# mpkuse/rgbd_odometry

Hardware: NVIDIA B200
Metric: frame-pairs aligned/s (640x480, 4-lvl) (higher is better)
Workload: dtype f32+f64

## Files before the change

### rgbd_odometry_b200/_lib.py

```python
import ctypes as C
import os

from . import build as _build

MAX_LEVELS = 6
STAGES = ["h2d", "pyramid", "canny", "edt_rows", "normgrad", "solve", "d2h"]


class Config(C.Structure):
    _fields_ = [("width", C.c_int), ("height", C.c_int), ("levels", C.c_int), ("max_batch", C.c_int), ("device", C.c_int),
                ("keep_now_depth", C.c_int), ("trace_iters", C.c_int)]


class SolverParams(C.Structure):
    _fields_ = [("solver", C.c_int), ("jacobian", C.c_int), ("weight", C.c_int), ("arithmetic", C.c_int),
                ("huber_k", C.c_float), ("lm_lambda0", C.c_double), ("iters", C.c_int * MAX_LEVELS), ("residual", C.c_int)]


class PairInfo(C.Structure):
    _fields_ = [("status", C.c_int), ("npts", C.c_int * MAX_LEVELS), ("best_index", C.c_int * MAX_LEVELS),
                ("iterations_run", C.c_int * MAX_LEVELS), ("best_energy", C.c_float * MAX_LEVELS),
                ("visible_ratio", C.c_float * MAX_LEVELS), ("laplacian_b", C.c_float)]


class CovInfo(C.Structure):
    _fields_ = [("status", C.c_int), ("level", C.c_int), ("nvis", C.c_int), ("sigma2", C.c_double), ("logdet", C.c_double)]


class PhotoConfig(C.Structure):
    _fields_ = [("width", C.c_int), ("height", C.c_int), ("levels", C.c_int), ("max_batch", C.c_int), ("device", C.c_int)]


class PhotoInfo(C.Structure):
    _fields_ = [("status", C.c_int), ("iters_run", C.c_int), ("nreproj", C.c_int), ("sumsq_first", C.c_double),
                ("sumsq_last", C.c_double), ("visible", C.c_double), ("A", C.c_double * 36), ("b", C.c_double * 6)]


class KeyframePolicy(C.Structure):
    _fields_ = [("keyframe_every", C.c_int), ("use_quality_gates", C.c_int), ("laplacian_thresh", C.c_float),
                ("visible_ratio_thresh", C.c_float), ("min_reprojections", C.c_int)]


RGBD_MAX_LEVELS = 5


class RgbdConfig(C.Structure):
    _fields_ = [("width", C.c_int), ("height", C.c_int), ("levels", C.c_int), ("max_batch", C.c_int), ("device", C.c_int)]


class RgbdParams(C.Structure):
    _fields_ = [("iterations", C.c_int), ("gradient_threshold", C.c_int), ("min_points", C.c_int), ("max_points", C.c_int),
                ("eps_norm_exit", C.c_double)]


class RgbdInfo(C.Structure):
    _fields_ = [("status", C.c_int), ("npts", C.c_int * RGBD_MAX_LEVELS), ("iters_run", C.c_int * RGBD_MAX_LEVELS),
                ("updates", C.c_int * RGBD_MAX_LEVELS), ("nvis_last", C.c_int * RGBD_MAX_LEVELS),
                ("eps_norm_first", C.c_double * RGBD_MAX_LEVELS), ("eps_norm_last", C.c_double * RGBD_MAX_LEVELS)]


SYMBOLS = [
    "dvo_last_error", "dvo_device_count", "dvo_create", "dvo_destroy", "dvo_set_stream", "dvo_synchronize",
    "dvo_set_intrinsics", "dvo_set_frames", "dvo_set_frames_raw", "dvo_promote_now_to_ref", "dvo_build_pyramids", "dvo_prepare",
    "dvo_set_initial_pose", "dvo_run", "dvo_process", "dvo_join", "dvo_join_stream", "dvo_get_poses", "dvo_align_batch", "dvo_level_dims", "dvo_get_level_buffer",
    "dvo_get_points", "dvo_eval_normal_equations", "dvo_eval_normal_equations_ex", "dvo_get_trace", "dvo_get_energies", "dvo_enable_timing", "dvo_get_stage_ms",
    "dvo_launch_count", "dvo_gop_compose", "dvo_run_sequences", "dvo_run_sequences_gated", "dvo_run_sequences_mem",
    "dvo_pose_covariance", "dvo_run_sequences_cov",
    "dvo_photo_create", "dvo_photo_destroy", "dvo_photo_set_stream", "dvo_photo_synchronize", "dvo_photo_launch_count",
    "dvo_photo_set_intrinsics", "dvo_photo_set_frames", "dvo_photo_prepare_ref", "dvo_photo_set_pose", "dvo_photo_estimate",
    "dvo_photo_get_poses", "dvo_photo_get_level", "dvo_photo_get_A", "dvo_photo_eval", "dvo_photo_put_level",
    "dvo_blob_create", "dvo_blob_upload", "dvo_blob_download", "dvo_blob_device_ptr", "dvo_blob_bytes", "dvo_blob_destroy",
    "dvo_undistort",
    "dvo_rgbd_create", "dvo_rgbd_destroy", "dvo_rgbd_set_stream", "dvo_rgbd_synchronize", "dvo_rgbd_launch_count",
    "dvo_rgbd_set_intrinsics", "dvo_rgbd_set_frames", "dvo_rgbd_compute_jacobians", "dvo_rgbd_set_pose", "dvo_rgbd_gauss_newton",
    "dvo_rgbd_get_poses", "dvo_rgbd_level_dims", "dvo_rgbd_get_level", "dvo_rgbd_get_A", "dvo_rgbd_eval",
]

_lib = None


def load(build_if_missing=True):
    global _lib
    if _lib is not None:
        return _lib
    path = _build.LIB
    if build_if_missing:
        path = _build.build_cuda()
    if not os.path.exists(path):
        raise RuntimeError(f"{path} is missing: build it with `python -m rgbd_odometry_b200.build` (no CPU fallback exists)")
    lib = C.CDLL(path)
    lib.dvo_last_error.restype = C.c_char_p
    lib.dvo_launch_count.restype = C.c_longlong
    lib.dvo_launch_count.argtypes = [C.c_void_p]
    lib.dvo_create.argtypes = [C.POINTER(Config), C.POINTER(C.c_void_p)]
    lib.dvo_destroy.argtypes = [C.c_void_p]
    lib.dvo_set_stream.argtypes = [C.c_void_p, C.c_void_p]
    lib.dvo_synchronize.argtypes = [C.c_void_p]
    lib.dvo_set_intrinsics.argtypes = [C.c_void_p, C.c_float, C.c_float, C.c_float, C.c_float]
    lib.dvo_set_frames.argtypes = [C.c_void_p, C.c_int, C.c_int, C.c_int, C.c_void_p, C.c_void_p, C.c_int]
    lib.dvo_set_frames_raw.argtypes = [C.c_void_p, C.c_int, C.c_int, C.c_int, C.c_void_p, C.c_void_p, C.c_int]
    lib.dvo_promote_now_to_ref.argtypes = [C.c_void_p, C.c_int, C.c_int]
    lib.dvo_build_pyramids.argtypes = [C.c_void_p, C.c_int, C.c_int, C.c_int]
    lib.dvo_prepare.argtypes = [C.c_void_p, C.c_int, C.c_int, C.c_int]
    lib.dvo_set_initial_pose.argtypes = [C.c_void_p, C.c_int, C.c_int, C.c_void_p, C.c_int]
    lib.dvo_run.argtypes = [C.c_void_p, C.c_int, C.c_int, C.POINTER(SolverParams)]
    lib.dvo_process.argtypes = [C.c_void_p, C.c_int, C.c_int, C.POINTER(SolverParams), C.c_void_p]
    lib.dvo_join.argtypes = [C.c_void_p]
    lib.dvo_join_stream.argtypes = [C.c_void_p, C.c_void_p]
    lib.dvo_get_poses.argtypes = [C.c_void_p, C.c_int, C.c_int, C.c_void_p, C.c_void_p, C.c_int]
    lib.dvo_align_batch.argtypes = [C.c_void_p, C.c_int, C.c_void_p, C.c_void_p, C.c_void_p, C.c_void_p,
                                    C.POINTER(SolverParams), C.c_void_p, C.c_void_p]
    lib.dvo_level_dims.argtypes = [C.c_void_p, C.c_int, C.POINTER(C.c_int), C.POINTER(C.c_int)]
    lib.dvo_get_level_buffer.argtypes = [C.c_void_p, C.c_int, C.c_int, C.c_int, C.c_int, C.c_void_p, C.c_size_t]
    lib.dvo_get_points.argtypes = [C.c_void_p, C.c_int, C.c_int, C.c_void_p, C.c_void_p, C.c_void_p, C.c_int, C.POINTER(C.c_int)]
    lib.dvo_eval_normal_equations.argtypes = [C.c_void_p, C.c_int, C.c_int, C.c_void_p, C.c_int, C.c_int, C.c_int, C.c_float,
                                              C.c_void_p, C.c_void_p, C.POINTER(C.c_double), C.POINTER(C.c_int),
                                              C.c_void_p, C.c_void_p, C.c_void_p, C.c_void_p, C.c_void_p]
    lib.dvo_eval_normal_equations_ex.argtypes = [C.c_void_p, C.c_int, C.c_int, C.c_void_p, C.POINTER(SolverParams),
                                                 C.c_void_p, C.c_void_p, C.POINTER(C.c_double), C.POINTER(C.c_int),
                                                 C.c_void_p, C.c_void_p, C.c_void_p, C.c_void_p, C.c_void_p]
    lib.dvo_get_trace.argtypes = [C.c_void_p, C.c_int, C.c_int, C.c_void_p]
    lib.dvo_get_energies.argtypes = [C.c_void_p, C.c_int, C.c_int, C.c_void_p, C.c_int]
    lib.dvo_enable_timing.argtypes = [C.c_void_p, C.c_int]
    lib.dvo_get_stage_ms.argtypes = [C.c_void_p, C.c_void_p]
    lib.dvo_gop_compose.argtypes = [C.c_void_p, C.c_int, C.c_int, C.c_void_p, C.c_void_p, C.c_void_p, C.c_int]
    lib.dvo_run_sequences.argtypes = [C.c_void_p, C.c_int, C.c_int, C.c_void_p, C.c_void_p, C.POINTER(SolverParams), C.c_int,
                                      C.c_void_p, C.c_void_p, C.c_void_p]
    lib.dvo_run_sequences_gated.argtypes = [C.c_void_p, C.c_int, C.c_int, C.c_void_p, C.c_void_p, C.POINTER(SolverParams),
                                            C.POINTER(KeyframePolicy), C.c_void_p, C.c_void_p, C.c_void_p, C.c_void_p]
    lib.dvo_run_sequences_mem.argtypes = [C.c_void_p, C.c_int, C.c_int, C.c_void_p, C.c_void_p, C.c_int, C.POINTER(SolverParams),
                                          C.POINTER(KeyframePolicy), C.c_void_p, C.c_void_p, C.c_void_p, C.c_void_p]
    lib.dvo_pose_covariance.argtypes = [C.c_void_p, C.c_int, C.c_int, C.POINTER(SolverParams), C.c_int, C.c_void_p, C.c_void_p, C.c_int]
    lib.dvo_run_sequences_cov.argtypes = [C.c_void_p, C.c_int, C.c_int, C.c_void_p, C.c_void_p, C.c_int, C.POINTER(SolverParams),
                                          C.POINTER(KeyframePolicy), C.c_void_p, C.c_void_p, C.c_void_p, C.c_void_p, C.c_void_p, C.c_void_p]
    lib.dvo_photo_create.argtypes = [C.POINTER(PhotoConfig), C.POINTER(C.c_void_p)]
    lib.dvo_photo_destroy.argtypes = [C.c_void_p]
    lib.dvo_photo_set_stream.argtypes = [C.c_void_p, C.c_void_p]
    lib.dvo_photo_synchronize.argtypes = [C.c_void_p]
    lib.dvo_photo_launch_count.restype = C.c_longlong
    lib.dvo_photo_launch_count.argtypes = [C.c_void_p]
    lib.dvo_photo_set_intrinsics.argtypes = [C.c_void_p, C.c_double, C.c_double, C.c_double, C.c_double]
    lib.dvo_photo_set_frames.argtypes = [C.c_void_p, C.c_int, C.c_int, C.c_int, C.c_void_p, C.c_void_p, C.c_int]
    lib.dvo_photo_prepare_ref.argtypes = [C.c_void_p, C.c_int, C.c_int, C.c_int]
    lib.dvo_photo_set_pose.argtypes = [C.c_void_p, C.c_int, C.c_int, C.c_void_p]
    lib.dvo_photo_estimate.argtypes = [C.c_void_p, C.c_int, C.c_int, C.c_int, C.c_int, C.c_int, C.c_double, C.c_double]
    lib.dvo_photo_get_poses.argtypes = [C.c_void_p, C.c_int, C.c_int, C.c_void_p, C.c_void_p]
    lib.dvo_photo_get_level.argtypes = [C.c_void_p, C.c_int, C.c_int, C.c_int, C.c_int, C.c_void_p, C.c_size_t, C.c_int]
    lib.dvo_photo_get_A.argtypes = [C.c_void_p, C.c_int, C.c_int, C.c_void_p]
    lib.dvo_photo_put_level.argtypes = [C.c_void_p, C.c_int, C.c_int, C.c_int, C.c_int, C.c_void_p, C.c_size_t]
    lib.dvo_blob_create.argtypes = [C.c_size_t, C.c_int, C.POINTER(C.c_void_p)]
    lib.dvo_blob_upload.argtypes = [C.c_void_p, C.c_void_p, C.c_size_t]
    lib.dvo_blob_download.argtypes = [C.c_void_p, C.c_void_p, C.c_size_t]
    lib.dvo_blob_device_ptr.argtypes = [C.c_void_p]
    lib.dvo_blob_device_ptr.restype = C.c_void_p
    lib.dvo_blob_bytes.argtypes = [C.c_void_p]
    lib.dvo_blob_bytes.restype = C.c_size_t
    lib.dvo_blob_destroy.argtypes = [C.c_void_p]
    lib.dvo_photo_eval.argtypes = [C.c_void_p, C.c_int, C.c_int, C.c_void_p, C.c_int, C.c_double, C.c_void_p, C.c_void_p,
                                   C.POINTER(C.c_double), C.POINTER(C.c_int), C.POINTER(C.c_int), C.c_void_p]
    lib.dvo_undistort.argtypes = [C.c_void_p, C.c_void_p, C.c_int, C.c_int, C.c_int, C.c_int, C.c_void_p, C.c_void_p, C.c_int, C.c_void_p]
    lib.dvo_rgbd_create.argtypes = [C.POINTER(RgbdConfig), C.POINTER(C.c_void_p)]
    lib.dvo_rgbd_destroy.argtypes = [C.c_void_p]
    lib.dvo_rgbd_set_stream.argtypes = [C.c_void_p, C.c_void_p]
    lib.dvo_rgbd_synchronize.argtypes = [C.c_void_p]
    lib.dvo_rgbd_launch_count.restype = C.c_longlong
    lib.dvo_rgbd_launch_count.argtypes = [C.c_void_p]
    lib.dvo_rgbd_set_intrinsics.argtypes = [C.c_void_p, C.c_double, C.c_double, C.c_double, C.c_double]
    lib.dvo_rgbd_set_frames.argtypes = [C.c_void_p, C.c_int, C.c_int, C.c_int, C.c_void_p, C.c_void_p, C.c_int]
    lib.dvo_rgbd_compute_jacobians.argtypes = [C.c_void_p, C.c_int, C.c_int, C.c_int]
    lib.dvo_rgbd_set_pose.argtypes = [C.c_void_p, C.c_int, C.c_int, C.c_void_p]
# ... 20 lines not shown
```

### rgbd_odometry_b200/build.py

```python
import os
import shutil
import subprocess

PKG = os.path.dirname(os.path.abspath(__file__))
ROOT = os.path.dirname(PKG)
CSRC = os.path.join(PKG, "csrc")
LIB = os.path.join(PKG, "libdvo_b200.so")
SYNTH_SRC = os.path.join(PKG, "synth", "synth.cpp")
SYNTH_LIB = os.path.join(PKG, "synth", "libdvo_synth.so")
HOST_DIR = os.path.join(PKG, "host")
HOST_LIB = os.path.join(PKG, "libdvo_host.so")


def _nvcc():
    for cand in (shutil.which("nvcc"), "/usr/local/cuda/bin/nvcc"):
        if cand and os.path.exists(cand):
            return cand
    raise RuntimeError("nvcc not found: libdvo_b200.so cannot be built and there is no CPU fallback")


def _stale(target, sources):
    if not os.path.exists(target):
        return True
    t = os.path.getmtime(target)
    return any(os.path.getmtime(s) > t for s in sources)


def cuda_sources():
    srcs = [os.path.join(CSRC, f) for f in sorted(os.listdir(CSRC)) if f.endswith(".cu")]
    deps = [os.path.join(CSRC, f) for f in sorted(os.listdir(CSRC)) if f.endswith(".cuh")]
    deps.append(os.path.join(ROOT, "include", "dvo_b200.h"))
    return srcs, deps


PER_FILE_FLAGS = {"photometric.cu": ["-fmad=false"], "rgbd.cu": ["-fmad=false"], "frontend.cu": ["-fmad=false"]}
COMPILE_FLAGS = ["-gencode", "arch=compute_100a,code=sm_100a", "-lineinfo", "-O3", "-std=c++17", "-Xcompiler", "-fPIC,-ffp-contract=off"]
OBJ_DIR = os.path.join(PKG, "build")


def build_cuda(force=False, verbose=False):
    srcs, deps = cuda_sources()
    os.makedirs(OBJ_DIR, exist_ok=True)
    objs, relink = [], force or not os.path.exists(LIB)
    for src in srcs:
        name = os.path.basename(src)
        obj = os.path.join(OBJ_DIR, name[:-3] + ".o")
        objs.append(obj)
        if force or _stale(obj, [src] + deps):
            extra = os.environ.get("DVO_NVCC_EXTRA", "").split()
            cmd = [_nvcc()] + COMPILE_FLAGS + PER_FILE_FLAGS.get(name, []) + extra + (["-Xptxas", "-v"] if verbose else []) + ["-c", "-o", obj, src]
            subprocess.check_call(cmd, cwd=CSRC)
            relink = True
    if relink or _stale(LIB, objs):
        subprocess.check_call([_nvcc(), "-gencode", "arch=compute_100a,code=sm_100a", "-shared", "-cudart", "static", "-o", LIB] + objs)
    return LIB


def build_synth(force=False):
    if force or _stale(SYNTH_LIB, [SYNTH_SRC]):
        subprocess.check_call(["g++", "-O2", "-std=c++17", "-fPIC", "-shared", "-pthread", "-o", SYNTH_LIB, SYNTH_SRC])
    return SYNTH_LIB


def build_host(force=False):
    if not os.path.isdir(HOST_DIR):
        return None
    srcs = [os.path.join(HOST_DIR, f) for f in sorted(os.listdir(HOST_DIR)) if f.endswith(".cpp")]
    if not srcs:
        return None
    deps = [os.path.join(HOST_DIR, f) for f in sorted(os.listdir(HOST_DIR)) if f.endswith(".h")]
    deps.append(os.path.join(ROOT, "include", "dvo_b200.h"))
    build_cuda()
    if force or _stale(HOST_LIB, srcs + deps + [LIB]):
        cmd = ["g++", "-O2", "-std=c++17", "-fPIC", "-shared", "-I", os.path.join(ROOT, "include"), "-I", HOST_DIR, "-o", HOST_LIB] + srcs + \
              ["-L", PKG, "-ldvo_b200", "-Wl,-rpath,$ORIGIN"]
        subprocess.check_call(cmd)
    return HOST_LIB


def build_all(force=False):
    build_cuda(force)
    build_synth(force)
    build_host(force)


if __name__ == "__main__":
    import sys
    build_all(force="--force" in sys.argv)
    print("built:", LIB)
```

### rgbd_odometry_b200/csrc/preprocess.cu

```cuda
#include <stdlib.h>

#include "common.cuh"

struct PyrArgs {
    PyrGeom g;
    uint8_t* gray;
    uint16_t* depth;
    int first;
    int sub_total;
    int l0;
    const unsigned char* active;
};

__global__ void __launch_bounds__(256) pyramid_nearest_kernel(PyrArgs a) {
    const int b = a.first + blockIdx.y;
    if (a.active && !a.active[b]) return;
    int q = blockIdx.x * blockDim.x + threadIdx.x;
    if (q >= a.sub_total) return;
    int l = a.l0;
    while (l < a.g.L - 1 && q >= a.g.P[l]) { q -= a.g.P[l]; ++l; }
    const int w = a.g.w[l], W0 = a.g.w[0], H0 = a.g.h[0];
    const int y = q / w, x = q - y * w;
    const int sy = min(y << l, H0 - 1), sx = min(x << l, W0 - 1);
    const long long src = lvl_at(a.g, 0, b) + (long long)sy * W0 + sx;
// ... 63 lines not shown
    uint32_t gv[4];
#pragma unroll
    for (int j = 0; j < 4; ++j) gv[j] = a.gray[row + sx[j]];
    if (a.depth) {
        uint32_t dv[4];
#pragma unroll
        for (int j = 0; j < 4; ++j) { dv[j] = a.depth[row + sx[j]]; }
#pragma unroll
        for (int j = 0; j < 4; ++j) dv[j] = dv[j] ? dv[j] : 1u;
        *reinterpret_cast<uint2*>(a.depth + dst) = make_uint2(dv[0] | (dv[1] << 16), dv[2] | (dv[3] << 16));
    }
    *reinterpret_cast<uint32_t*>(a.gray + dst) = gv[0] | (gv[1] << 8) | (gv[2] << 16) | (gv[3] << 24);
}

int launch_pyramid(dvo_ctx* c, int first, int count, int frames_mask) {
    const PyrGeom& g = c->geom;
    if (g.L < 2) return DVO_OK;
    const bool vec1 = (g.w[0] == 2 * g.w[1]) && (g.w[1] % 4 == 0);
    const int l0 = vec1 ? 2 : 1;
    int sub = 0;
    bool vec_rest = true;
    for (int l = l0; l < g.L; ++l) { sub += g.P[l]; vec_rest = vec_rest && (g.w[l] % 4 == 0) && (g.off[l] % 4 == 0) && (g.P[l] % 4 == 0); }
    for (int f = 0; f < 2; ++f) {
        if (!(frames_mask & (1 << f))) continue;
        PyrArgs a; a.g = g; a.gray = c->gray[f]; a.depth = c->depth[f]; a.first = first; a.sub_total = sub; a.l0 = l0; a.active = c->active;
        if (vec1 && g.w[1] % 8 == 0 && g.off[1] % 8 == 0 && g.P[1] % 8 == 0 && g.P[0] % 16 == 0) {
            dim3 grid1((g.P[1] / 8 + 255) / 256, count);
            pyramid_level1_vec8_kernel<<<grid1, 256, 0, c->stream>>>(a);
            c->launches++;
        } else if (vec1) {
            dim3 grid1((g.P[1] / 4 + 255) / 256, count);
            pyramid_level1_vec4_kernel<<<grid1, 256, 0, c->stream>>>(a);
            c->launches++;
        }
        if (sub > 0 && vec_rest) {
            dim3 grid((sub / 4 + 255) / 256, count);
            pyramid_nearest_vec4_kernel<<<grid, 256, 0, c->stream>>>(a);
            c->launches++;
        } else if (sub > 0) {
            dim3 grid((sub + 255) / 256, count);
            pyramid_nearest_kernel<<<grid, 256, 0, c->stream>>>(a);
            c->launches++;
        }
    }
    DVO_CUDA(cudaGetLastError());
    return DVO_OK;
}

struct CannyArgs {
    const uint8_t* gray[2];
    uint8_t* edge[2];
    const uint16_t* depth;
    uint16_t* gcol;
    float *X, *Y, *Z;
    int* pix;
    int* npts;
    unsigned* nedge[2];
    int w, h, P, L;
    int frame0;
    int count;
    long long gscratch_frame_stride;
    float tmpfx, tmpfy, tmpcx, tmpcy;
    uint32_t* gscratch;
    long long gscratch_stride;
    int first;
    int bm_words;
    const unsigned char* active;
};

__device__ __forceinline__ void sobel3(const uint8_t* __restrict__ g, int w, int h, int y, int x, int& dx, int& dy) {
    const int ym = max(y - 1, 0), yp = min(y + 1, h - 1), xm = max(x - 1, 0), xp = min(x + 1, w - 1);
    const uint8_t* r0 = g + ym * w; const uint8_t* r1 = g + y * w; const uint8_t* r2 = g + yp * w;
    const int a = r0[xm], b = r0[x], c = r0[xp], d = r1[xm], f = r1[xp], p = r2[xm], q = r2[x], r = r2[xp];
    dx = (c + 2 * f + r) - (a + 2 * d + p);
    dy = (p + 2 * q + r) - (a + 2 * b + c);
}
__device__ __forceinline__ int mag_at(const uint8_t* __restrict__ g, int w, int h, int y, int x) {
    if ((unsigned)y >= (unsigned)h || (unsigned)x >= (unsigned)w) return 0;
    int dx, dy; sobel3(g, w, h, y, x, dx, dy);
    return dx * dx + dy * dy;
}

__device__ __forceinline__ uint32_t expand4(uint32_t nib) { return (((nib & 0xFu) * 0x00204081u) & 0x01010101u) * 0xFFu; }

__device__ __forceinline__ void row_sums(const uint8_t* __restrict__ grow, int w, int x, int lane, int& hs, int& hb) {
    const int v = (x < w) ? (int)grow[x] : 0;
    int l = __shfl_up_sync(0xffffffffu, v, 1), r = __shfl_down_sync(0xffffffffu, v, 1);
    if (lane == 0) l = (x > 0 && x < w) ? (int)grow[x - 1] : v;
    if (lane == 31) r = (x + 1 < w) ? (int)grow[x + 1] : v;
    if (x + 1 >= w) r = v;
    hs = r - l; hb = l + 2 * v + r;
}

#ifndef DVO_NMS_L2_AHEAD
#define DVO_NMS_L2_AHEAD 4
#endif
#ifndef DVO_NMS_MIN_BLOCKS
#define DVO_NMS_MIN_BLOCKS 2
#endif
#ifndef DVO_NMS_ROWS
#define DVO_NMS_ROWS 48
#endif
#ifndef DVO_NMS_WARPS
#define DVO_NMS_WARPS 8
#endif
constexpr int NMS_ROWS = DVO_NMS_ROWS, NMS_WARPS = DVO_NMS_WARPS;
struct NmsArgs {
    const uint8_t* gray[2];
    uint32_t* scratch;
    long long slot_stride, frame_stride;
    long long off[DVO_MAX_LEVELS];
    long long bm_off[DVO_MAX_LEVELS];
    int w[DVO_MAX_LEVELS], h[DVO_MAX_LEVELS], P[DVO_MAX_LEVELS], bm_words[DVO_MAX_LEVELS];
    int chunks[DVO_MAX_LEVELS], strips[DVO_MAX_LEVELS], task_end[DVO_MAX_LEVELS];
    int L, first, count, frame0;
    float low, high;
    const unsigned char* active;
};
struct NmsSums { float s[4], b[4], sH, bH; };
struct NmsMags { float m[4], L, R; };
struct NmsGrad { float dx[4], dy[4]; };

template <bool VEC>
__global__ void __launch_bounds__(NMS_WARPS * 32, DVO_NMS_MIN_BLOCKS) sobel_nms_kernel(NmsArgs a) {
    const int lane = threadIdx.x & 31;
    int task = blockIdx.x * NMS_WARPS + (threadIdx.x >> 5);
    int l = 0;
    while (l < a.L && task >= a.task_end[l]) ++l;
    if (l >= a.L) return;
    if (l) task -= a.task_end[l - 1];
    const int chunks = a.chunks[l], strips = a.strips[l];
    const int chunk = task % chunks, t2 = task / chunks, strip = t2 % strips, img = t2 / strips;
    const int second = (img >= a.count) ? 1 : 0;
    const int frame = second ? DVO_FRAME_NOW : a.frame0;
    const int b = a.first + img - second * a.count;
    if (a.active && !a.active[b]) return;
    const int w = a.w[l], h = a.h[l];
    const int wd = (w + 31) >> 5, pitch = wd + 2;
    const uint8_t* __restrict__ g = a.gray[frame] + a.off[l] + (long long)b * a.P[l];
    uint32_t* Cb = a.scratch + (long long)b * a.slot_stride + (long long)frame * a.frame_stride + a.bm_off[l];
    const int bmw = a.bm_words[l];
    const int c0 = chunk << 7, xb = c0 + (lane << 2);
    const int y0 = strip * NMS_ROWS, y1 = min(h, y0 + NMS_ROWS);
    const bool first_lane = (lane == 0), last_lane = (lane == 31);
    const bool halo_valid = first_lane ? (c0 > 0) : (last_lane && c0 + 128 < w);
    const bool self_left = (xb == 0), self_right = (xb + 4 >= w);
    const int hx0 = first_lane ? c0 - 2 : c0 + 128;
    const uint32_t sel_near = 0x7440u + (first_lane ? 1u : 0u), sel_far = 0x7440u + (first_lane ? 0u : 1u);
    const float lowt = (xb < w) ? a.low : 3.0e38f, high = a.high;
    const float K = 13573.0f / 32768.0f;

    const bool in_image = (xb < w);
    const uint8_t* __restrict__ gx = g + (in_image ? xb : 0);
    const uint8_t* __restrict__ gh = g + (halo_valid ? hx0 : 0);
    const unsigned roff_max = (unsigned)((h - 1) * w);
    auto load_row = [&](unsigned roff, uint32_t& wv, uint32_t& hv) {
        if (VEC) {
            wv = in_image ? *reinterpret_cast<const uint32_t*>(gx + roff) : 0u;
            hv = halo_valid ? (uint32_t)*reinterpret_cast<const uint16_t*>(gh + roff) : 0u;
        } else {
            const uint8_t* __restrict__ row = g + roff;
            wv = 0u;
#pragma unroll
            for (int j = 0; j < 4; ++j) wv |= (uint32_t)row[min(xb + j, w - 1)] << (8 * j);
            hv = halo_valid ? ((uint32_t)row[hx0] | ((uint32_t)row[min(hx0 + 1, w - 1)] << 8)) : 0u;
        }
    };
    auto byte_f = [](uint32_t wv, uint32_t sel) { return __uint_as_float(__byte_perm(wv, 0x4B000000u, sel)) - 8388608.0f; };
    auto sums = [&](uint32_t wv, uint32_t hv, NmsSums& S) {
        float v[4];
#pragma unroll
        for (int j = 0; j < 4; ++j) v[j] = byte_f(wv, 0x7440u + j);
        const float hn = byte_f(hv, sel_near), hf = byte_f(hv, sel_far);
        float lft = __shfl_up_sync(0xffffffffu, v[3], 1), rgt = __shfl_down_sync(0xffffffffu, v[0], 1);
        if (first_lane) lft = hn;
        if (last_lane) rgt = hn;
        if (self_left) lft = v[0];
        if (self_right) rgt = v[3];
        S.s[0] = v[1] - lft;  S.s[1] = v[2] - v[0]; S.s[2] = v[3] - v[1]; S.s[3] = rgt - v[2];
        S.b[0] = fmaf(2.0f, v[0], lft) + v[1];  S.b[1] = fmaf(2.0f, v[1], v[0]) + v[2];
        S.b[2] = fmaf(2.0f, v[2], v[1]) + v[3]; S.b[3] = fmaf(2.0f, v[3], v[2]) + rgt;
        const float gm1 = first_lane ? hf : v[3], gp1 = first_lane ? v[0] : hf;
        S.sH = gp1 - gm1; S.bH = fmaf(2.0f, hn, gm1) + gp1;
    };
    auto grad_mag = [&](bool inside, const NmsSums& A, const NmsSums& B, const NmsSums& Cs, NmsGrad& G, NmsMags& M) {
        float mH;
        if (inside) {
#pragma unroll
            for (int j = 0; j < 4; ++j) {
                G.dx[j] = fmaf(2.0f, B.s[j], A.s[j]) + Cs.s[j]; G.dy[j] = Cs.b[j] - A.b[j];
                M.m[j] = fmaf(G.dx[j], G.dx[j], G.dy[j] * G.dy[j]);
            }
            const float dxH = fmaf(2.0f, B.sH, A.sH) + Cs.sH, dyH = Cs.bH - A.bH;
            mH = halo_valid ? fmaf(dxH, dxH, dyH * dyH) : 0.0f;
            if (!VEC) {
#pragma unroll
                for (int j = 0; j < 4; ++j) if (xb + j >= w) M.m[j] = 0.0f;
            }
        } else {
#pragma unroll
            for (int j = 0; j < 4; ++j) { G.dx[j] = 0.0f; G.dy[j] = 0.0f; M.m[j] = 0.0f; }
            mH = 0.0f;
        }
        M.L = __shfl_up_sync(0xffffffffu, M.m[3], 1); M.R = __shfl_down_sync(0xffffffffu, M.m[0], 1);
        if (first_lane) M.L = mH;
// ... 4 lines not shown
    uint32_t wv, hv;
    NmsSums S0, S1, S2;
    NmsMags M0, M1, M2;
    NmsGrad G0, G1;
    auto row_off = [&](int r) { return min((unsigned)max(r, 0) * (unsigned)w, roff_max); };
    load_row(row_off(y0 - 2), wv, hv); sums(wv, hv, S0);
    load_row(row_off(y0 - 1), wv, hv); sums(wv, hv, S1);
    load_row(row_off(y0), wv, hv);     sums(wv, hv, S2);
    grad_mag(y0 > 0, S0, S1, S2, G0, M0);
    load_row(row_off(y0 + 1), wv, hv); sums(wv, hv, S0);
    grad_mag(true, S1, S2, S0, G0, M1);
    uint32_t wvn, hvn;
    load_row(row_off(y0 + 2), wvn, hvn);
    unsigned roff_next = row_off(y0 + 3);
    unsigned roff_l2 = row_off(y0 + 3 + DVO_NMS_L2_AHEAD);

    const int widx = (c0 >> 5) + (lane >> 3);
    const bool writer = ((lane & 7) == 0) && widx < wd;
    uint32_t* Cp = Cb + (long long)(y0 + 1) * pitch + 1 + widx;
    const int sh = (lane & 3) << 2;

    auto nms_row = [&](const NmsMags& P, const NmsMags& C, const NmsMags& N, const NmsGrad& Gc) {
        float crm[4], ncm[4];
#pragma unroll
        for (int j = 0; j < 4; ++j) { crm[j] = ((j < 3) ? C.m[j < 3 ? j + 1 : 3] : C.R) - 0.5f; ncm[j] = N.m[j] - 0.5f; }
        uint32_t bits = 0u;
#pragma unroll
        for (int j = 0; j < 4; ++j) {
            const float m = C.m[j];
            const float cl = j ? C.m[j > 0 ? j - 1 : 0] : C.L;
            const float pl = j ? P.m[j > 0 ? j - 1 : 0] : P.L, pr = (j < 3) ? P.m[j < 3 ? j + 1 : 3] : P.R;
            const float nl = j ? N.m[j > 0 ? j - 1 : 0] : N.L, nr = (j < 3) ? N.m[j < 3 ? j + 1 : 3] : N.R;
            const float adx = fabsf(Gc.dx[j]), ady = fabsf(Gc.dy[j]);
            const float t = adx * K, u = fmaf(adx, -2.0f, ady);
            const bool horiz = ady < t, vert = u > t;
            const bool neg = Gc.dx[j] * Gc.dy[j] < 0.0f;
            const float da = neg ? pr : pl, db = neg ? nl : nr;
            const float na = horiz ? cl : (vert ? P.m[j] : da);
            const float nb = horiz ? crm[j] : (vert ? ncm[j] : db);
            const bool cand = (m > na) && (m > nb) && (m > lowt);
            const bool strong = cand && (m > high);
            bits |= (cand ? (1u << j) : 0u) | (strong ? (0x10000u << j) : 0u);
        }
        bits <<= sh;
        bits |= __shfl_xor_sync(0xffffffffu, bits, 1);
        bits |= __shfl_xor_sync(0xffffffffu, bits, 2);
        const uint32_t hi = __shfl_down_sync(0xffffffffu, bits, 4);
        if (writer) {
            Cp[0] = __byte_perm(bits, hi, 0x5410);
            Cp[bmw] = __byte_perm(bits, hi, 0x7632);
        }
        Cp += pitch;
    };
    auto row_step = [&](const NmsSums& A, const NmsSums& B, NmsSums& Cs, const NmsMags& P, const NmsMags& C, NmsMags& N,
                        const NmsGrad& Gc, NmsGrad& Gn) {
        wv = wvn; hv = hvn;
        load_row(roff_next, wvn, hvn); roff_next = min(roff_next + (unsigned)w, roff_max);
        if (DVO_NMS_L2_AHEAD > 0) {
            if (in_image) asm volatile("prefetch.global.L2 [%0];" :: "l"(gx + roff_l2));
            roff_l2 = min(roff_l2 + (unsigned)w, roff_max);
        }
        sums(wv, hv, Cs);
        grad_mag(true, A, B, Cs, Gn, N);
        nms_row(P, C, N, Gc);
    };
    const int yend = (y1 == h) ? y1 - 1 : y1;
    int y = y0;
    for (; y + 6 <= yend; y += 6) {
        row_step(S2, S0, S1, M0, M1, M2, G0, G1);
        row_step(S0, S1, S2, M1, M2, M0, G1, G0);
        row_step(S1, S2, S0, M2, M0, M1, G0, G1);
        row_step(S2, S0, S1, M0, M1, M2, G1, G0);
        row_step(S0, S1, S2, M1, M2, M0, G0, G1);
        row_step(S1, S2, S0, M2, M0, M1, G1, G0);
    }
    for (; y < yend; ++y) {
        row_step(S2, S0, S1, M0, M1, M2, G0, G1);
        S2 = S0; S0 = S1; M0 = M1; M1 = M2; G0 = G1;
    }
    if (y1 == h) {
        grad_mag(false, S2, S0, S1, G1, M2);
        nms_row(M0, M1, M2, G0);
    }
}

constexpr int CANNY_MAX_WARPS = 24;
#ifndef DVO_CANNY_INTERLEAVE
#define DVO_CANNY_INTERLEAVE 1
#endif
#ifndef DVO_CANNY_STOP_AFTER
#define DVO_CANNY_STOP_AFTER 0
#endif

template <bool GLOBAL_BITMAPS> struct HystPtr { typedef volatile uint32_t* type; };
template <> struct HystPtr<true> { typedef uint32_t* type; };

template <bool GLOBAL_BITMAPS>
__global__ void __launch_bounds__(768, 2) canny_kernel(CannyArgs a) {
    extern __shared__ uint32_t smem_u32[];
    __shared__ int s_scan[CANNY_MAX_WARPS + 1];
    __shared__ int s_base;
    __shared__ unsigned s_cnt;
    __shared__ unsigned char s_chg[2][768];
    const int T = blockDim.x;
    const int tid = threadIdx.x, lane = tid & 31, warp = tid >> 5;
#if DVO_CANNY_INTERLEAVE
    const bool both = a.count != 0x7fffffff;
    const int second = both ? (int)(blockIdx.x & 1u) : 0;
    const int frame = second ? DVO_FRAME_NOW : a.frame0;
    const int b = a.first + (both ? (int)(blockIdx.x >> 1) : (int)blockIdx.x);
#else
    const int second = (blockIdx.x >= (unsigned)a.count) ? 1 : 0;
    const int frame = second ? DVO_FRAME_NOW : a.frame0;
    const int b = a.first + (int)blockIdx.x - second * a.count;
#endif
    const bool do_points = (frame == DVO_FRAME_REF), do_cols = (frame == DVO_FRAME_NOW);
    if (a.active && !a.active[b]) return;
    const int w = a.w, h = a.h;
    const int wd = (w + 31) >> 5, pitch = wd + 2;
    const int nwords = a.bm_words;
    uint32_t* C = GLOBAL_BITMAPS ? a.gscratch + (long long)b * a.gscratch_stride + (long long)frame * a.gscratch_frame_stride : smem_u32;
    uint32_t* E = C + nwords;

    if (GLOBAL_BITMAPS) {
        for (int i = tid; i < pitch; i += T) { C[i] = 0u; E[i] = 0u; C[(h + 1) * pitch + i] = 0u; E[(h + 1) * pitch + i] = 0u; }
        for (int y = tid; y < h; y += T) {
            C[(y + 1) * pitch] = 0u; E[(y + 1) * pitch] = 0u; C[(y + 1) * pitch + wd + 1] = 0u; E[(y + 1) * pitch + wd + 1] = 0u;
        }
    } else {
        const uint32_t* __restrict__ src = a.gscratch + (long long)b * a.gscratch_stride + (long long)frame * a.gscratch_frame_stride;
        if ((reinterpret_cast<uintptr_t>(src) & 15) == 0 && (nwords & 1) == 0) {
            const uint4* s4 = reinterpret_cast<const uint4*>(src); uint4* d4 = reinterpret_cast<uint4*>(C);
            for (int i = tid; i < (nwords >> 1); i += T) d4[i] = s4[i];
        } else {
            for (int i = tid; i < 2 * nwords; i += T) C[i] = src[i];
        }
    }
    if (tid == 0) { s_cnt = 0u; s_base = 0; }
    __syncthreads();

#if DVO_CANNY_STOP_AFTER == 1
    return;
#endif
    {
        const int Hs = max(1, min(h, min(T, 768) / wd));
        const int Rh = (h + Hs - 1) / Hs;
        const int items = wd * Hs;
        const int sh = tid / wd, wx = tid - sh * wd;
        const bool owner = tid < items;
        const int ya = sh * Rh, yb = min(h, ya + Rh);
        for (int i = tid; i < 2 * 768; i += T) (&s_chg[0][0])[i] = (i < 768) ? 1 : 0;
        __syncthreads();
        int cur = 0;
        for (;;) {
            int changed = 0;
            bool active = false;
            if (owner && ya < yb) {
                for (int dsy = -1; dsy <= 1 && !active; ++dsy)
                    for (int dwx = -1; dwx <= 1; ++dwx) {
                        const int s2 = sh + dsy, w2 = wx + dwx;
                        if (s2 >= 0 && s2 < Hs && w2 >= 0 && w2 < wd && s_chg[cur][s2 * wd + w2]) { active = true; break; }
                    }
            }
            if (active) {
                auto spread = [](uint32_t l, uint32_t c, uint32_t r) { return c | (c << 1) | (c >> 1) | (l >> 31) | (r << 31); };
                auto flood = [](uint32_t f, uint32_t c) {
                    const uint32_t up = ((c + f) ^ c) & c;
                    const uint32_t cr = __brev(c), fr = __brev(f);
                    return f | up | __brev(((cr + fr) ^ cr) & cr);
                };
                typename HystPtr<GLOBAL_BITMAPS>::type Ev = E;
                const uint32_t* Cv = C;
                {
                    int idx = (ya + 1) * pitch + wx + 1;
                    uint32_t sp = spread(Ev[idx - pitch - 1], Ev[idx - pitch], Ev[idx - pitch + 1]);
                    uint32_t el = Ev[idx - 1], ec = Ev[idx], er = Ev[idx + 1];
                    for (int y = ya; y < yb; ++y, idx += pitch) {
                        const uint32_t nl = Ev[idx + pitch - 1], nc = Ev[idx + pitch], nr = Ev[idx + pitch + 1];
                        const uint32_t c = Cv[idx];
                        uint32_t f = ec;
                        if (c != 0u && ec != c) {
                            f = flood(ec | (c & (sp | spread(el, ec, er) | spread(nl, nc, nr))), c);
                            if (f != ec) { Ev[idx] = f; changed = 1; }
                        }
                        sp = spread(el, f, er); el = nl; ec = nc; er = nr;
                    }
                }
                {
                    int idx = yb * pitch + wx + 1;
                    uint32_t sp = spread(Ev[idx + pitch - 1], Ev[idx + pitch], Ev[idx + pitch + 1]);
                    uint32_t el = Ev[idx - 1], ec = Ev[idx], er = Ev[idx + 1];
                    for (int y = yb - 1; y >= ya; --y, idx -= pitch) {
                        const uint32_t nl = Ev[idx - pitch - 1], nc = Ev[idx - pitch], nr = Ev[idx - pitch + 1];
                        const uint32_t c = Cv[idx];
                        uint32_t f = ec;
                        if (c != 0u && ec != c) {
                            f = flood(ec | (c & (sp | spread(el, ec, er) | spread(nl, nc, nr))), c);
                            if (f != ec) { Ev[idx] = f; changed = 1; }
                        }
                        sp = spread(el, f, er); el = nl; ec = nc; er = nr;
                    }
                }
            }
            if (owner) s_chg[cur ^ 1][tid] = (unsigned char)changed;
            cur ^= 1;
            if (!__syncthreads_or(changed)) break;
        }
    }

#if DVO_CANNY_STOP_AFTER == 2
    return;
#endif
    const int nw = h * wd;
    {
        uint8_t* eo = a.edge[frame] + (long long)b * a.P;
        unsigned cnt = 0;
        const bool vec_ok = (w % 16 == 0) && ((reinterpret_cast<uintptr_t>(eo) & 15) == 0);
        for (int q = tid; q < nw; q += T) {
            const int y = q / wd, wx = q - y * wd;
            const uint32_t e = E[(y + 1) * pitch + wx + 1];
            cnt += __popc(e);
            const int x0 = wx << 5;
            if (vec_ok && x0 + 32 <= w) {
                uint4 v0, v1;
                v0.x = expand4(e); v0.y = expand4(e >> 4); v0.z = expand4(e >> 8); v0.w = expand4(e >> 12);
                v1.x = expand4(e >> 16); v1.y = expand4(e >> 20); v1.z = expand4(e >> 24); v1.w = expand4(e >> 28);
                uint4* dst = reinterpret_cast<uint4*>(eo + (long long)y * w + x0);
                dst[0] = v0; dst[1] = v1;
            } else {
                for (int i = 0; i < 32 && x0 + i < w; ++i) eo[(long long)y * w + x0 + i] = ((e >> i) & 1u) ? 255 : 0;
            }
        }
        for (int o = 16; o > 0; o >>= 1) cnt += __shfl_down_sync(0xffffffffu, cnt, o);
        if (lane == 0 && cnt) atomicAdd(&s_cnt, cnt);
    }

#if DVO_CANNY_STOP_AFTER == 3
    return;
#endif
    if (do_points) {
        const uint16_t* __restrict__ dep = a.depth + (long long)b * a.P;
        for (int q = tid; q < nw; q += T) {
            const int y = q / wd, wx = q - y * wd;
            const int idx = (y + 1) * pitch + wx + 1;
            uint32_t e = E[idx], sel = 0u;
            const uint16_t* __restrict__ dr = dep + (long long)y * w + (wx << 5);
            while (e) {
                const int i0 = __ffs(e) - 1; e &= e - 1;
                const int i1 = e ? __ffs(e) - 1 : i0; e &= e - 1;
                const int i2 = e ? __ffs(e) - 1 : i0; e &= e - 1;
                const int i3 = e ? __ffs(e) - 1 : i0; e &= e - 1;
                const unsigned d0 = dr[i0], d1 = dr[i1], d2 = dr[i2], d3 = dr[i3];
                sel |= (d0 > 100u ? 1u << i0 : 0u) | (d1 > 100u ? 1u << i1 : 0u) | (d2 > 100u ? 1u << i2 : 0u) | (d3 > 100u ? 1u << i3 : 0u);
            }
            E[idx] = sel;
        }
    }
    __syncthreads();
    if (tid == 0) a.nedge[frame][(long long)b * a.L] = s_cnt;

    const int hw = (h + 31) >> 5, hwp = hw | 1;
    uint32_t* Et = C;
    if (do_cols) {
        const int nwarps = T >> 5;
        for (int blk = warp; blk < hw * wd; blk += nwarps) {
            const int wy = blk / wd, wx = blk - wy * wd;
            const int y = (wy << 5) + lane;
            const uint32_t word = (y < h) ? E[(y + 1) * pitch + wx + 1] : 0u;
            uint32_t mine = 0u;
#pragma unroll
            for (int j = 0; j < 32; ++j) { const uint32_t bt = __ballot_sync(0xffffffffu, (word >> j) & 1u); if (lane == j) mine = bt; }
            Et[((wx << 5) + lane) * hwp + wy] = mine;
        }
    }
    __syncthreads();

    if (do_cols) {
        uint16_t* gc = a.gcol + (long long)b * a.P;
        const int BIG = 1 << 20;
        for (int x = tid; x < w; x += T) {
            const uint32_t* col = Et + x * hwp;
            int lastrow = -BIG;
            int nextrow = -1;
            for (int wy = 0; wy < hw; ++wy) {
                const uint32_t Wd = col[wy];
                const int base = wy << 5;
                if (nextrow < base + 32) {
                    nextrow = BIG;
                    for (int kk = wy + 1; kk < hw; ++kk) { const uint32_t vv = col[kk]; if (vv) { nextrow = (kk << 5) + __ffs(vv) - 1; break; } }
                }
                uint16_t* o = gc + (long long)base * w + x;
#pragma unroll
                for (int bt = 0; bt < 32; ++bt) {
                    if (base + bt < h) {
                        const uint32_t mle = Wd & (0xffffffffu >> (31 - bt));
                        const uint32_t mge = Wd & (0xffffffffu << bt);
                        const int dn = mle ? bt - (31 - __clz(mle)) : base + bt - lastrow;
                        const int up = mge ? (__ffs(mge) - 1) - bt : nextrow - (base + bt);
                        o[(long long)bt * w] = (uint16_t)min(min(dn, up), DVO_EDT_INF_1D);
                    }
                }
                if (Wd) lastrow = base + 31 - __clz(Wd);
            }
        }
    }

    if (do_points) {
        const uint16_t* __restrict__ dep = a.depth + (long long)b * a.P;
        float* X = a.X + (long long)b * a.P; float* Y = a.Y + (long long)b * a.P; float* Z = a.Z + (long long)b * a.P;
        int* pix = a.pix + (long long)b * a.P;
        const int per = (nw + T - 1) / T;
        const int q0 = min(nw, tid * per), q1 = min(nw, q0 + per);
        int mycnt = 0;
        for (int q = q0; q < q1; ++q) { const int y = q / wd, wx = q - y * wd; mycnt += __popc(E[(y + 1) * pitch + wx + 1]); }
        int incl = mycnt;
        for (int o = 1; o < 32; o <<= 1) { const int t = __shfl_up_sync(0xffffffffu, incl, o); if (lane >= o) incl += t; }
        if (lane == 31) s_scan[warp] = incl;
        __syncthreads();
        if (tid < 32) {
            const int nwp = T >> 5;
            const int v = (tid < nwp) ? s_scan[tid] : 0;
            int iv = v;
            for (int o = 1; o < 32; o <<= 1) { const int t = __shfl_up_sync(0xffffffffu, iv, o); if (lane >= o) iv += t; }
            if (tid < nwp) s_scan[tid] = iv - v;
            if (tid == 31) s_scan[CANNY_MAX_WARPS] = iv;
        }
        __syncthreads();
        int off = s_scan[warp] + (incl - mycnt);
        for (int q = q0; q < q1; ++q) {
            const int y = q / wd, wx = q - y * wd;
            uint32_t v = E[(y + 1) * pitch + wx + 1];
            const uint16_t* __restrict__ dr = dep + (long long)y * w;
            while (v) {
                int xs[4], n = 0;
#pragma unroll
                for (int k = 0; k < 4; ++k) {
                    if (v) { xs[k] = (wx << 5) + __ffs(v) - 1; v &= v - 1; n = k + 1; } else xs[k] = xs[0];
                }
                unsigned dv[4];
#pragma unroll
                for (int k = 0; k < 4; ++k) dv[k] = dr[xs[k]];
#pragma unroll
                for (int k = 0; k < 4; ++k) {
                    if (k < n) {
                        const int x = xs[k];
                        const float z = __fdiv_rn((float)dv[k], 1000.0f);
                        X[off + k] = __fmul_rn(__fmul_rn(z, __fsub_rn((float)x, a.tmpcx)), a.tmpfx);
                        Y[off + k] = __fmul_rn(__fmul_rn(z, __fsub_rn((float)y, a.tmpcy)), a.tmpfy);
                        Z[off + k] = z;
                        pix[off + k] = y * w + x;
                    }
                }
                off += n;
            }
        }
        if (tid == 0) a.npts[(long long)b * a.L] = s_scan[CANNY_MAX_WARPS];
    }
}

static int canny_bitmap_words(int w, int h) {
    const int wd = (w + 31) >> 5;
    const int a = (wd + 2) * (h + 2);
    const int t = (wd << 5) * (((h + 31) >> 5) | 1);
    return a > t ? a : t;
}

void canny_scratch_layout(const PyrGeom& g, long long* bm_off, int* bm_words, size_t* words_per_image) {
    long long o = 0;
    for (int l = 0; l < g.L; ++l) { bm_off[l] = o; bm_words[l] = canny_bitmap_words(g.w[l], g.h[l]); o += 2LL * ((bm_words[l] + 3) & ~3); }
    *words_per_image = (size_t)o;
}

int launch_canny(dvo_ctx* c, int first, int count, int frames_mask) {
    const PyrGeom& g = c->geom;
    if (!(frames_mask & 3)) return DVO_OK;
    if ((frames_mask & 1) && !c->depth[0]) { dvo_set_error("canny: reference depth missing"); return DVO_ERR_STATE; }
    if (!c->bitmap_scratch) { dvo_set_error("canny: bitmap scratch missing"); return DVO_ERR_STATE; }
    const bool both = (frames_mask & 3) == 3;
    const int frame0 = (frames_mask & 1) ? DVO_FRAME_REF : DVO_FRAME_NOW;
    const long long slot_stride = (long long)c->bitmap_scratch_words, frame_stride = slot_stride * g.Bmax;
    {
        NmsArgs n;
        n.gray[0] = c->gray[0]; n.gray[1] = c->gray[1];
        n.scratch = c->bitmap_scratch; n.slot_stride = slot_stride; n.frame_stride = frame_stride;
        long long tasks = 0;
// ... 687 lines not shown
```

Baseline: 102,200.

## Use incremental column distance transform and add optional in-tile hysteresis closure

The column 1D distance pass now keeps running down-distance and next-edge counters instead of doing clz/ffs mask math for every pixel, and it splits full and partial 32-row blocks so the full case stays unrolled. A warp-level tile closure for hysteresis is added to the NMS kernel, but it only runs when DVO_NMS_CLOSE_SWEEPS is above zero, which it is not by default. The spread/flood helpers move to file scope, and a build helper for variant libraries is added. The active change targets per-pixel bit work in the EDT column pass and adds a serial dependency chain per pixel in its place.

```diff
diff --git a/rgbd_odometry_b200/_lib.py b/rgbd_odometry_b200/_lib.py
--- a/rgbd_odometry_b200/_lib.py
+++ b/rgbd_odometry_b200/_lib.py
@@ -79,13 +79,14 @@
 _lib = None
 
 
-def load(build_if_missing=True):
+def load(build_if_missing=True, path=None):
     global _lib
     if _lib is not None:
+        if path is not None and path != _lib._name:
+            raise RuntimeError(f"{_lib._name} is already loaded in this process; {path} cannot be loaded beside it")
         return _lib
-    path = _build.LIB
-    if build_if_missing:
-        path = _build.build_cuda()
+    if path is None:
+        path = _build.build_cuda() if build_if_missing else _build.LIB
     if not os.path.exists(path):
         raise RuntimeError(f"{path} is missing: build it with `python -m rgbd_odometry_b200.build` (no CPU fallback exists)")
     lib = C.CDLL(path)
diff --git a/rgbd_odometry_b200/build.py b/rgbd_odometry_b200/build.py
--- a/rgbd_odometry_b200/build.py
+++ b/rgbd_odometry_b200/build.py
@@ -56,6 +56,24 @@
     return LIB
 
 
+def build_cuda_variant(out_dir, extra, files=("preprocess.cu",)):
+    build_cuda()
+    os.makedirs(out_dir, exist_ok=True)
+    srcs, _ = cuda_sources()
+    objs = []
+    for src in srcs:
+        name = os.path.basename(src)
+        obj = os.path.join(OBJ_DIR, name[:-3] + ".o")
+        if name in files:
+            obj = os.path.join(out_dir, name[:-3] + ".o")
+            cmd = [_nvcc()] + COMPILE_FLAGS + PER_FILE_FLAGS.get(name, []) + list(extra) + ["-c", "-o", obj, src]
+            subprocess.check_call(cmd, cwd=CSRC)
+        objs.append(obj)
+    lib = os.path.join(out_dir, "libdvo_b200.so")
+    subprocess.check_call([_nvcc(), "-gencode", "arch=compute_100a,code=sm_100a", "-shared", "-cudart", "static", "-o", lib] + objs)
+    return lib
+
+
 def build_synth(force=False):
     if force or _stale(SYNTH_LIB, [SYNTH_SRC]):
         subprocess.check_call(["g++", "-O2", "-std=c++17", "-fPIC", "-shared", "-pthread", "-o", SYNTH_LIB, SYNTH_SRC])
diff --git a/rgbd_odometry_b200/csrc/preprocess.cu b/rgbd_odometry_b200/csrc/preprocess.cu
--- a/rgbd_odometry_b200/csrc/preprocess.cu
+++ b/rgbd_odometry_b200/csrc/preprocess.cu
@@ -169,6 +169,13 @@
 }
 
 __device__ __forceinline__ uint32_t expand4(uint32_t nib) { return (((nib & 0xFu) * 0x00204081u) & 0x01010101u) * 0xFFu; }
+
+__device__ __forceinline__ uint32_t hyst_spread(uint32_t l, uint32_t c, uint32_t r) { return c | (c << 1) | (c >> 1) | (l >> 31) | (r << 31); }
+__device__ __forceinline__ uint32_t hyst_flood(uint32_t f, uint32_t c) {
+    const uint32_t up = ((c + f) ^ c) & c;
+    const uint32_t cr = __brev(c), fr = __brev(f);
+    return f | up | __brev(((cr + fr) ^ cr) & cr);
+}
 
 __device__ __forceinline__ void row_sums(const uint8_t* __restrict__ grow, int w, int x, int lane, int& hs, int& hb) {
     const int v = (x < w) ? (int)grow[x] : 0;
@@ -208,6 +215,75 @@
 struct NmsMags { float m[4], L, R; };
 struct NmsGrad { float dx[4], dy[4]; };
 
+#ifndef DVO_NMS_CLOSE_SWEEPS
+#define DVO_NMS_CLOSE_SWEEPS 0
+#endif
+constexpr int NMS_SEG_ROWS = NMS_ROWS / 8;
+static_assert(NMS_ROWS % 8 == 0, "the tile closure splits a tile into 8 row segments");
+
+__device__ __forceinline__ void nms_tile_closure(uint32_t* tile, int pitch, int bmw, int rows, int words, int lane) {
+    constexpr int S = NMS_SEG_ROWS;
+    const int col = lane & 3, seg = lane >> 2;
+    const uint32_t ml = (col > 0) ? ~0u : 0u, mr = (col < 3) ? ~0u : 0u;
+    const uint32_t ma = (seg > 0) ? ~0u : 0u, mb = (seg < 7) ? ~0u : 0u;
+    uint32_t* p = tile + (long long)seg * S * pitch + col;
+    uint32_t c[S], e[S];
+    uint32_t weak = 0u, strong = 0u;
+#pragma unroll
+    for (int k = 0; k < S; ++k) {
+        const bool ok = col < words && seg * S + k < rows;
+        c[k] = ok ? p[k * pitch] : 0u;
+        e[k] = ok ? p[k * pitch + bmw] : 0u;
+        weak |= c[k] & ~e[k]; strong |= e[k];
+    }
+    if (!__any_sync(0xffffffffu, weak != 0u) || !__any_sync(0xffffffffu, strong != 0u)) return;
+    uint32_t dirty = 0u;
+    auto step = [&](int k, uint32_t al, uint32_t ac, uint32_t ar, uint32_t bl, uint32_t bc, uint32_t br, bool& changed) {
+        const uint32_t el = __shfl_up_sync(0xffffffffu, e[k], 1) & ml, er = __shfl_down_sync(0xffffffffu, e[k], 1) & mr;
+        const uint32_t f = hyst_flood(e[k] | (c[k] & hyst_spread(al | el | bl, ac | e[k] | bc, ar | er | br)), c[k]);
+        if (f != e[k]) { changed = true; dirty |= 1u << k; }
+        e[k] = f;
+    };
+    auto above = [&](int k, uint32_t& l, uint32_t& cc, uint32_t& r) {
+        if (k > 0) {
+            cc = e[k - 1];
+            l = __shfl_up_sync(0xffffffffu, cc, 1) & ml; r = __shfl_down_sync(0xffffffffu, cc, 1) & mr;
+        } else {
+            cc = __shfl_up_sync(0xffffffffu, e[S - 1], 4) & ma;
+            l = __shfl_up_sync(0xffffffffu, e[S - 1], 5) & ma & ml; r = __shfl_up_sync(0xffffffffu, e[S - 1], 3) & ma & mr;
+        }
+    };
+    auto below = [&](int k, uint32_t& l, uint32_t& cc, uint32_t& r) {
+        if (k < S - 1) {
+            cc = e[k + 1];
+            l = __shfl_up_sync(0xffffffffu, cc, 1) & ml; r = __shfl_down_sync(0xffffffffu, cc, 1) & mr;
+        } else {
+            cc = __shfl_down_sync(0xffffffffu, e[0], 4) & mb;
+            l = __shfl_down_sync(0xffffffffu, e[0], 3) & mb & ml; r = __shfl_down_sync(0xffffffffu, e[0], 5) & mb & mr;
+        }
+    };
+#pragma unroll 1
+    for (int it = 0; it < DVO_NMS_CLOSE_SWEEPS; ++it) {
+        bool changed = false;
+#pragma unroll
+        for (int k = 0; k < S; ++k) {
+            uint32_t al, ac, ar, bl, bc, br;
+            above(k, al, ac, ar); below(k, bl, bc, br);
+            step(k, al, ac, ar, bl, bc, br, changed);
+        }
+#pragma unroll
+        for (int k = S - 1; k >= 0; --k) {
+            uint32_t al, ac, ar, bl, bc, br;
+            above(k, al, ac, ar); below(k, bl, bc, br);
+            step(k, al, ac, ar, bl, bc, br, changed);
+        }
+        if (!__any_sync(0xffffffffu, changed)) break;
+    }
+#pragma unroll
+    for (int k = 0; k < S; ++k)
+        if (dirty & (1u << k)) p[k * pitch + bmw] = e[k];
+}
+
 template <bool VEC>
 __global__ void __launch_bounds__(NMS_WARPS * 32, DVO_NMS_MIN_BLOCKS) sobel_nms_kernel(NmsArgs a) {
     const int lane = threadIdx.x & 31;
@@ -378,6 +454,10 @@
         grad_mag(false, S2, S0, S1, G1, M2);
         nms_row(M0, M1, M2, G0);
     }
+    if (DVO_NMS_CLOSE_SWEEPS > 0) {
+        __syncwarp();
+        nms_tile_closure(Cb + (long long)(y0 + 1) * pitch + 1 + (c0 >> 5), pitch, bmw, y1 - y0, wd - (c0 >> 5), lane);
+    }
 }
 
 constexpr int CANNY_MAX_WARPS = 24;
@@ -459,42 +539,36 @@
                     }
             }
             if (active) {
-                auto spread = [](uint32_t l, uint32_t c, uint32_t r) { return c | (c << 1) | (c >> 1) | (l >> 31) | (r << 31); };
-                auto flood = [](uint32_t f, uint32_t c) {
-                    const uint32_t up = ((c + f) ^ c) & c;
-                    const uint32_t cr = __brev(c), fr = __brev(f);
-                    return f | up | __brev(((cr + fr) ^ cr) & cr);
-                };
                 typename HystPtr<GLOBAL_BITMAPS>::type Ev = E;
                 const uint32_t* Cv = C;
                 {
                     int idx = (ya + 1) * pitch + wx + 1;
-                    uint32_t sp = spread(Ev[idx - pitch - 1], Ev[idx - pitch], Ev[idx - pitch + 1]);
+                    uint32_t sp = hyst_spread(Ev[idx - pitch - 1], Ev[idx - pitch], Ev[idx - pitch + 1]);
                     uint32_t el = Ev[idx - 1], ec = Ev[idx], er = Ev[idx + 1];
                     for (int y = ya; y < yb; ++y, idx += pitch) {
                         const uint32_t nl = Ev[idx + pitch - 1], nc = Ev[idx + pitch], nr = Ev[idx + pitch + 1];
                         const uint32_t c = Cv[idx];
                         uint32_t f = ec;
                         if (c != 0u && ec != c) {
-                            f = flood(ec | (c & (sp | spread(el, ec, er) | spread(nl, nc, nr))), c);
+                            f = hyst_flood(ec | (c & (sp | hyst_spread(el, ec, er) | hyst_spread(nl, nc, nr))), c);
                             if (f != ec) { Ev[idx] = f; changed = 1; }
                         }
-                        sp = spread(el, f, er); el = nl; ec = nc; er = nr;
+                        sp = hyst_spread(el, f, er); el = nl; ec = nc; er = nr;
                     }
                 }
                 {
                     int idx = yb * pitch + wx + 1;
-                    uint32_t sp = spread(Ev[idx + pitch - 1], Ev[idx + pitch], Ev[idx + pitch + 1]);
+                    uint32_t sp = hyst_spread(Ev[idx + pitch - 1], Ev[idx + pitch], Ev[idx + pitch + 1]);
                     uint32_t el = Ev[idx - 1], ec = Ev[idx], er = Ev[idx + 1];
                     for (int y = yb - 1; y >= ya; --y, idx -= pitch) {
                         const uint32_t nl = Ev[idx - pitch - 1], nc = Ev[idx - pitch], nr = Ev[idx - pitch + 1];
                         const uint32_t c = Cv[idx];
                         uint32_t f = ec;
                         if (c != 0u && ec != c) {
-                            f = flood(ec | (c & (sp | spread(el, ec, er) | spread(nl, nc, nr))), c);
+                            f = hyst_flood(ec | (c & (sp | hyst_spread(el, ec, er) | hyst_spread(nl, nc, nr))), c);
                             if (f != ec) { Ev[idx] = f; changed = 1; }
                         }
-                        sp = spread(el, f, er); el = nl; ec = nc; er = nr;
+                        sp = hyst_spread(el, f, er); el = nl; ec = nc; er = nr;
                     }
                 }
             }
@@ -576,8 +650,9 @@
         const int BIG = 1 << 20;
         for (int x = tid; x < w; x += T) {
             const uint32_t* col = Et + x * hwp;
-            int lastrow = -BIG;
+            int dn = BIG;
             int nextrow = -1;
+            int nb = -1;
             for (int wy = 0; wy < hw; ++wy) {
                 const uint32_t Wd = col[wy];
                 const int base = wy << 5;
@@ -585,18 +660,24 @@
                     nextrow = BIG;
                     for (int kk = wy + 1; kk < hw; ++kk) { const uint32_t vv = col[kk]; if (vv) { nextrow = (kk << 5) + __ffs(vv) - 1; break; } }
                 }
+                if (nb < base) nb = Wd ? base + __ffs(Wd) - 1 : nextrow;
                 uint16_t* o = gc + (long long)base * w + x;
-#pragma unroll
-                for (int bt = 0; bt < 32; ++bt) {
-                    if (base + bt < h) {
-                        const uint32_t mle = Wd & (0xffffffffu >> (31 - bt));
-                        const uint32_t mge = Wd & (0xffffffffu << bt);
-                        const int dn = mle ? bt - (31 - __clz(mle)) : base + bt - lastrow;
-                        const int up = mge ? (__ffs(mge) - 1) - bt : nextrow - (base + bt);
-                        o[(long long)bt * w] = (uint16_t)min(min(dn, up), DVO_EDT_INF_1D);
+                auto pixel = [&](int bt) {
+                    const bool edge = (Wd >> bt) & 1u;
+                    dn = edge ? 0 : dn + 1;
+                    *o = (uint16_t)min(min(dn, nb - (base + bt)), DVO_EDT_INF_1D);
+                    o += w;
+                    if (edge) {
+                        const uint32_t m = (bt < 31) ? (Wd & (0xfffffffeu << bt)) : 0u;
+                        nb = m ? base + __ffs(m) - 1 : nextrow;
                     }
+                };
+                if (base + 32 <= h) {
+#pragma unroll
+                    for (int bt = 0; bt < 32; ++bt) pixel(bt);
+                } else {
+                    for (int bt = 0; bt < h - base; ++bt) pixel(bt);
                 }
-                if (Wd) lastrow = base + 31 - __clz(Wd);
             }
         }
     }
```

Result: faster. 103,700 (median of 6 runs) (+1.5%).
